# cheukwaylee/ORB_SLAM2_detailed_comments

Measured on AMD Instinct MI355X. Metric: frames/sec ORB extract+match (1000 kp, 640x480), higher is better.
Workload: dtype u8; 1 GPU; synthetic 640x480 mono stream, nFeatures=1000, 8 levels, scale 1.2, FAST 20/7, extract+match(t vs t-1), batch 1024 frames/GPU resident in HBM, 1 pipelines/GPU; parallelism=single GPU

## Files before the change

orb_slam2_detailed_comments_amd/csrc/orbx_kernels.hip:

```cpp
#include "orbx_device.h"
#include "orbx_inplace.h"
#include "orbx_fast_net.h"
#include "orbx_track.h"
#include "../../include/orbx_pattern_data.h"

#define L0_ROWS 8
#ifndef L0_FF
#define L0_FF 1
#endif
#ifndef RR_FF
#define RR_FF 1
#endif
#define QT_KPT ORBX_QT_KPT
#ifndef QT_DROP_STAGE_A
#define QT_DROP_STAGE_A 1
#endif
#ifndef QT_ONE_SCAN
#define QT_ONE_SCAN 1
#endif
#ifndef QT_REG_SIZE
#define QT_REG_SIZE 1
#endif
#ifndef QT_CENSUS_NODES
#define QT_CENSUS_NODES 1
// ... 1918 lines not shown
            const int r = __mul24(i, 13108) >> 16, q8 = i - r * (DS_HC / 8);
            const uint32_t *w = patch + r * (DS_PP / 4) + 2 * q8;
            const uint32_t w0 = w[0], w1 = w[1], w2 = w[2], w3 = w[3];
            const uint32_t KLO = 18u | (34u << 8) | (49u << 16) | (55u << 24), KHI = 49u | (34u << 8) | (18u << 16);
            uint32_t hv[8];
            hv[0] = __builtin_amdgcn_udot4(w0, KLO, __builtin_amdgcn_udot4(w1, KHI, 0u, false), false);
            hv[4] = __builtin_amdgcn_udot4(w1, KLO, __builtin_amdgcn_udot4(w2, KHI, 0u, false), false);
#pragma unroll
            for (int j = 1; j < 4; ++j) {
                const uint32_t a01 = __builtin_amdgcn_alignbyte(w1, w0, j), a12 = __builtin_amdgcn_alignbyte(w2, w1, j),
                               a23 = __builtin_amdgcn_alignbyte(w3, w2, j);
                hv[j] = __builtin_amdgcn_udot4(a01, KLO, __builtin_amdgcn_udot4(a12, KHI, 0u, false), false);
                hv[4 + j] = __builtin_amdgcn_udot4(a12, KLO, __builtin_amdgcn_udot4(a23, KHI, 0u, false), false);
            }
            uint4 o;
            o.x = hv[0] | (hv[1] << 16);
            o.y = hv[2] | (hv[3] << 16);
            o.z = hv[4] | (hv[5] << 16);
            o.w = hv[6] | (hv[7] << 16);
            *(uint4 *)(hrow + r * DS_HC + 8 * q8) = o;
        }
#endif
        __builtin_amdgcn_fence(__ATOMIC_RELEASE, "wavefront");
        __builtin_amdgcn_wave_barrier();
        __builtin_amdgcn_fence(__ATOMIC_ACQUIRE, "wavefront");
        if (dbg_stop == 3) return;
        const float factorPI = (float)(3.1415926535897932384626433832795 / 180.f);
        const float angle = angle_deg * factorPI;
                const OrbxSinCos sc = orbx_sincosf_pinned(angle);
        const float a = sc.c, b = sc.s;
        const int wvec = (L.pw - 2 * L.org) & ~3;
#if DS_PATTERN_F32
#define DS_PX(t) (((t) & 1) ? patf[(t) >> 1].z : patf[(t) >> 1].x)
#define DS_PY(t) (((t) & 1) ? patf[(t) >> 1].w : patf[(t) >> 1].y)
#else
        const int pw4[4] = {pat.x, pat.y, pat.z, pat.w};
#define DS_PX(t) ((float)(signed char)((pw4[(t) >> 1] >> (16 * ((t) & 1))) & 0xff))
#define DS_PY(t) ((float)(signed char)((pw4[(t) >> 1] >> (16 * ((t) & 1) + 8)) & 0xff))
#endif
        unsigned long long words[4];
        if (x + (DS_R - 3) < wvec) {
#if DS_COLFIRST
            const uint32_t cbias = (uint32_t)(2 * ((DS_R - 3) * DS_VC + (DS_R - 3))) - 0x400000u * (2u * DS_VC) - (0x4B400000u << 1);
#else
            const uint32_t cbias = (uint32_t)(2 * ((DS_R - 3) * DS_HC + (DS_R - 3))) - 0x400000u * (2u * DS_HC) - (0x4B400000u << 1);
#endif
            const uint32_t hbase = (uint32_t)(uintptr_t)(orbx_lds_u16p)hrow + cbias;
            float tv[8];
            float nb = -b;
            asm("" : "+v"(nb));
#pragma unroll
            for (int t0 = 0; t0 < 8; t0 += DS_TAP_BATCH) {
                uint32_t adr[DS_TAP_BATCH], I[DS_TAP_BATCH];
#pragma unroll
                for (int k = 0; k < DS_TAP_BATCH; ++k) {
                    const float px = DS_PX(t0 + k), py = DS_PY(t0 + k);
                    float fy, fx;
                    if (FPM == ORBX_FP_GCC_FMA) {
                        fy = __builtin_fmaf(px, b, py * a);
                        fx = __builtin_fmaf(px, a, py * nb);
                    } else {
                        fy = px * b + py * a;
                        fx = px * a + py * nb;
                    }
                    const uint32_t uy = __float_as_uint(fy + 12582912.0f), ux = __float_as_uint(fx + 12582912.0f);
#if DS_COLFIRST
#if DS_MFMA
                    uint32_t ay = (uy << 1) + hbase;
                    asm("" : "+v"(ay));
                    adr[k] = __umul24(ux, 2u * DS_VC) + ay;
#else
                    adr[k] = __umul24(uy, 2u * DS_VC) + ((ux << 1) + hbase);
#endif
#else
                    adr[k] = __umul24(uy, 2u * DS_HC) + ((ux << 1) + hbase);
                    asm("" : "+v"(adr[k]));
#endif
                }
#if DS_COLFIRST
                orbx_ds_taps<DS_TAP_BATCH>(adr, I);
#else
#pragma unroll
                for (int k = 0; k < DS_TAP_BATCH; ++k) {
                    const orbx_lds_u16p hp = (orbx_lds_u16p)(uintptr_t)adr[k];
                    const uint32_t r0 = hp[3 * DS_HC], r1 = (uint32_t)hp[2 * DS_HC] + hp[4 * DS_HC],
                                   r2 = (uint32_t)hp[1 * DS_HC] + hp[5 * DS_HC], r3 = (uint32_t)hp[0] + hp[6 * DS_HC];
                    I[k] = __umul24(55u, r0) + __umul24(49u, r1) + __umul24(34u, r2) + __umul24(18u, r3);
                }
#endif
#pragma unroll
                for (int k = 0; k < DS_TAP_BATCH; ++k) tv[t0 + k] = __builtin_fminf(__builtin_rintf((float)I[k] * (1.f / 65536.f)), 255.f);
            }
#pragma unroll
            for (int r = 0; r < 4; ++r) words[r] = orbx_ballot(tv[2 * r] < tv[2 * r + 1]);
        } else {
            int tval[8];
#pragma unroll
            for (int t0 = 0; t0 < 8; t0 += DS_TAP_BATCH) {
                uint32_t adr[DS_TAP_BATCH], I[DS_TAP_BATCH];
                int ixs[DS_TAP_BATCH];
#pragma unroll
                for (int k = 0; k < DS_TAP_BATCH; ++k) {
                    const float px = DS_PX(t0 + k), py = DS_PY(t0 + k);
                    float fy, fx;
                    if (FPM == ORBX_FP_GCC_FMA) {
                        fy = __builtin_fmaf(px, b, py * a);
                        fx = __builtin_fmaf(px, a, -(py * b));
                    } else {
                        fy = px * b + py * a;
                        fx = px * a - py * b;
                    }
                    const int iy = (int)__builtin_rintf(fy), ix = (int)__builtin_rintf(fx);
                    ixs[k] = ix;
#if DS_COLFIRST
#if DS_MFMA
                    adr[k] = (uint32_t)(uintptr_t)(orbx_lds_u16p)hrow + 2u * (uint32_t)(__mul24(ix + DS_R - 3, DS_VC) + (iy + DS_R - 3));
#else
                    adr[k] = (uint32_t)(uintptr_t)(orbx_lds_u16p)hrow + 2u * (uint32_t)(__mul24(iy + DS_R - 3, DS_VC) + (ix + DS_R - 3));
#endif
#else
                    adr[k] = (uint32_t)(__mul24(iy + DS_R - 3, DS_HC) + (ix + DS_R - 3));
#endif
                }
#if DS_COLFIRST
                orbx_ds_taps<DS_TAP_BATCH>(adr, I);
#else
#pragma unroll
                for (int k = 0; k < DS_TAP_BATCH; ++k) {
                    const uint16_t *hp = hrow + adr[k];
                    const uint32_t r0 = hp[3 * DS_HC], r1 = (uint32_t)hp[2 * DS_HC] + hp[4 * DS_HC],
                                   r2 = (uint32_t)hp[1 * DS_HC] + hp[5 * DS_HC], r3 = (uint32_t)hp[0] + hp[6 * DS_HC];
                    I[k] = __umul24(55u, r0) + __umul24(49u, r1) + __umul24(34u, r2) + __umul24(18u, r3);
                }
#endif
#pragma unroll
                for (int k = 0; k < DS_TAP_BATCH; ++k) {
                    const uint32_t tie = x + ixs[k] >= wvec ? 1u : ((I[k] >> 16) & 1u);
                    tval[t0 + k] = (int)min((I[k] + 0x7fffu + tie) >> 16, 255u);
                }
            }
#pragma unroll
            for (int r = 0; r < 4; ++r) words[r] = orbx_ballot(tval[2 * r] < tval[2 * r + 1]);
        }
        if (lane < 4) {
            unsigned long long w = lane == 0 ? words[0] : lane == 1 ? words[1] : lane == 2 ? words[2] : words[3];
            *(unsigned long long *)(desc + ((long long)f * cap + oi) * 32 + 8 * lane) = w;
        }
        if (lane == 0) {
            orbx_keypoint kp;
            float fx = (float)x, fy = (float)y;
            if (level != 0) { fx = fx * L.scale; fy = fy * L.scale; }
            kp.x = fx; kp.y = fy;
            kp.size = L.size;
            kp.angle = angle_deg;
            kp.response = (float)(pos >> 24);
            kp.octave = level;
            kp.class_id = -1;
            kps[(long long)f * cap + oi] = kp;
        }
    }
}

#define MT_SPLIT 16
#define MT_WAVES 4
#define MT_QPW(QT) (32 * (QT))
#define MT_QPB(QT) (MT_WAVES * MT_QPW(QT))
#define MT_CHUNK 4096
typedef int mt_v4i __attribute__((ext_vector_type(4)));
typedef int mt_v16i __attribute__((ext_vector_type(16)));
__device__ __forceinline__ uint32_t mt_min2(uint32_t a, uint32_t b) { return a < b ? a : b; }
__device__ __forceinline__ uint32_t mt_max2(uint32_t a, uint32_t b) { return a > b ? a : b; }
template <int QT>
__global__ __launch_bounds__(64 * MT_WAVES, QT == 2 ? 3 : 2) void k_match(const uint8_t *__restrict__ q, const int *__restrict__ nq,
                                                         long long q_stride, const uint8_t *__restrict__ t,
                                                         const int *__restrict__ nt, long long t_stride,
                                                         uint2 *__restrict__ partial, int *__restrict__ best_idx,
                                                         int *__restrict__ best_dist, int *__restrict__ second_dist,
                                                         int out_stride, int nsplit) {
    __shared__ __attribute__((aligned(16))) int s_tk[MT_CHUNK];
    const int lane = threadIdx.x & 63, w = __builtin_amdgcn_readfirstlane(threadIdx.x >> 6), pr = blockIdx.z, sp = blockIdx.y;
    const int NQ = min(nq[pr], out_stride), NT = min(nt[pr], 1 << 20);
    if ((int)blockIdx.x * MT_QPB(QT) >= NQ) return;
    const int r = lane & 31, h = lane >> 5;
    const uint8_t *qp = q + (long long)pr * q_stride;
    const uint8_t *tp = t + (long long)pr * t_stride;
    const int per = ((NT + 31) / 32 + nsplit - 1) / nsplit * 32;
    const int j0 = min(NT, sp * per), j1 = min(NT, j0 + per);
    const int qw = blockIdx.x * MT_QPB(QT) + w * MT_QPW(QT);
    const bool wave_on = qw < NQ;
    mt_v4i bq[QT][8];
    int pq[QT];
#pragma unroll
    for (int c = 0; c < QT; ++c) {
        const int qi = qw + 32 * c + r;
        uint4 v = make_uint4(0, 0, 0, 0);
        if (qi < NQ) v = *(const uint4 *)(qp + (long long)qi * 32 + 16 * h);
        pq[c] = __popc(v.x) + __popc(v.y) + __popc(v.z) + __popc(v.w);
        pq[c] += __shfl_xor(pq[c], 32);
#pragma unroll
        for (int p = 0; p < 8; ++p) {
            bq[c][p][0] = (int)((v.x << (7 - p)) & 0x80808080u);
            bq[c][p][1] = (int)((v.y << (7 - p)) & 0x80808080u);
            bq[c][p][2] = (int)((v.z << (7 - p)) & 0x80808080u);
            bq[c][p][3] = (int)((v.w << (7 - p)) & 0x80808080u);
        }
    }
    uint32_t gbest[QT], gsecond[QT];
#pragma unroll
    for (int c = 0; c < QT; ++c) gbest[c] = gsecond[c] = 0xffffffffu;
    for (int c0 = j0; c0 < j1; c0 += MT_CHUNK) {
        const int c1 = min(j1, c0 + MT_CHUNK), n = c1 - c0, npad = (n + 31) & ~31;
        __syncthreads();
        for (int i = threadIdx.x; i < npad; i += 64 * MT_WAVES) {
            int key = 0x7fffffff;
            if (i < n) {
                const uint4 a = *(const uint4 *)(tp + (long long)(c0 + i) * 32), b = *(const uint4 *)(tp + (long long)(c0 + i) * 32 + 16);
                const int pt = __popc(a.x) + __popc(a.y) + __popc(a.z) + __popc(a.w) + __popc(b.x) + __popc(b.y) + __popc(b.z) + __popc(b.w);
                key = ((pt + 256) << 12) | i;
            }
            s_tk[i] = key;
        }
        __syncthreads();
        if (!wave_on) continue;
        int best[QT], second[QT];
#pragma unroll
        for (int c = 0; c < QT; ++c) best[c] = second[c] = 0x7fffffff;
        const uint8_t *trow = tp + (long long)(c0 + r) * 32 + 16 * h;
        uint4 ta = make_uint4(0, 0, 0, 0);
        if (r < n) ta = *(const uint4 *)trow;
        for (int jt = 0; jt < npad; jt += 32) {
            const uint4 tc = ta;
            ta = make_uint4(0, 0, 0, 0);
            if (jt + 32 + r < n) ta = *(const uint4 *)(trow + (long long)(jt + 32) * 32);
            mt_v16i acc[QT];
            {
                const int4 *kp = (const int4 *)(s_tk + jt + 4 * h);
#pragma unroll
                for (int g = 0; g < 4; ++g) {
                    const int4 k4 = kp[2 * g];
                    acc[0][4 * g] = k4.x; acc[0][4 * g + 1] = k4.y; acc[0][4 * g + 2] = k4.z; acc[0][4 * g + 3] = k4.w;
                }
#pragma unroll
                for (int c = 1; c < QT; ++c) acc[c] = acc[0];
            }
#pragma unroll
            for (int p = 0; p < 8; ++p) {
                mt_v4i a;
                if (p < 6) {
                    a[0] = (int)((tc.x << (6 - p)) & 0x40404040u); a[1] = (int)((tc.y << (6 - p)) & 0x40404040u);
                    a[2] = (int)((tc.z << (6 - p)) & 0x40404040u); a[3] = (int)((tc.w << (6 - p)) & 0x40404040u);
                } else if (p == 6) {
                    a[0] = (int)(tc.x & 0x40404040u); a[1] = (int)(tc.y & 0x40404040u);
                    a[2] = (int)(tc.z & 0x40404040u); a[3] = (int)(tc.w & 0x40404040u);
                } else {
                    a[0] = (int)((tc.x >> 1) & 0x40404040u); a[1] = (int)((tc.y >> 1) & 0x40404040u);
                    a[2] = (int)((tc.z >> 1) & 0x40404040u); a[3] = (int)((tc.w >> 1) & 0x40404040u);
                }
#pragma unroll
                for (int c = 0; c < QT; ++c) acc[c] = __builtin_amdgcn_mfma_i32_32x32x32_i8(a, bq[c][p], acc[c], 0, 0, 0);
            }
#pragma unroll
            for (int i = 0; i < 16; ++i) {
#pragma unroll
                for (int c = 0; c < QT; ++c) {
                    const int kc = acc[c][i];
                    second[c] = max(min(best[c], second[c]), min(max(best[c], second[c]), kc));
                    best[c] = min(best[c], kc);
                }
            }
        }
#pragma unroll
        for (int c = 0; c < QT; ++c) {
            const uint32_t b = best[c] == 0x7fffffff ? 0xffffffffu
                                                     : ((uint32_t)((best[c] >> 12) + pq[c] - 256) << 20) | (uint32_t)(c0 + (best[c] & 4095));
            const uint32_t s2 = second[c] == 0x7fffffff ? 0xffffffffu
                                                        : ((uint32_t)((second[c] >> 12) + pq[c] - 256) << 20) | (uint32_t)(c0 + (second[c] & 4095));
            gsecond[c] = mt_min2(mt_min2(gsecond[c], s2), mt_max2(gbest[c], b));
            gbest[c] = mt_min2(gbest[c], b);
        }
    }
    if (!wave_on) return;
#pragma unroll
    for (int c = 0; c < QT; ++c) {
        const uint32_t ob = (uint32_t)__shfl_xor((int)gbest[c], 32), os = (uint32_t)__shfl_xor((int)gsecond[c], 32);
        const uint32_t second = mt_min2(mt_min2(gsecond[c], os), mt_max2(gbest[c], ob));
        const uint32_t best = mt_min2(gbest[c], ob);
        const int qi = qw + 32 * c + r;
        if (h == 0 && qi < NQ) {
            if (nsplit > 1) {
                partial[((long long)pr * nsplit + sp) * out_stride + qi] = make_uint2(best, second);
            } else {
                const long long o = (long long)pr * out_stride + qi;
                best_idx[o] = best == 0xffffffffu ? -1 : (int)(best & 0xfffffu);
                best_dist[o] = best == 0xffffffffu ? 0x7fffffff : (int)(best >> 20);
                second_dist[o] = second == 0xffffffffu ? 0x7fffffff : (int)(second >> 20);
            }
        }
    }
}

typedef int mt_v8i __attribute__((ext_vector_type(8)));
typedef float mt_v16f __attribute__((ext_vector_type(16)));
#define MT_F4_NONE 0x7f7fffff
#ifndef MT_F4_LB2
#define MT_F4_LB2 3
#endif
#ifndef MT_F4_LB4
#define MT_F4_LB4 2
#endif
#ifndef MT_F4_USE4
#define MT_F4_USE4 1
#endif
template <int QT>
__global__ __launch_bounds__(64 * MT_WAVES, QT == 2 ? MT_F4_LB2 : MT_F4_LB4) void k_match_f4(const uint8_t *__restrict__ q, const int *__restrict__ nq,
                                                         long long q_stride, const uint8_t *__restrict__ t,
                                                         const int *__restrict__ nt, long long t_stride,
                                                         uint2 *__restrict__ partial, int *__restrict__ best_idx,
                                                         int *__restrict__ best_dist, int *__restrict__ second_dist,
                                                         int out_stride, int nsplit) {
    __shared__ __attribute__((aligned(16))) float s_tk[MT_CHUNK];
    const int lane = threadIdx.x & 63, w = __builtin_amdgcn_readfirstlane(threadIdx.x >> 6), pr = blockIdx.z, sp = blockIdx.y;
    const int NQ = min(nq[pr], out_stride), NT = min(nt[pr], 1 << 20);
    if ((int)blockIdx.x * MT_QPB(QT) >= NQ) return;
    const int r = lane & 31, h = lane >> 5;
    const uint8_t *qp = q + (long long)pr * q_stride;
    const uint8_t *tp = t + (long long)pr * t_stride;
    const int per = ((NT + 31) / 32 + nsplit - 1) / nsplit * 32;
    const int j0 = min(NT, sp * per), j1 = min(NT, j0 + per);
    const int qw = blockIdx.x * MT_QPB(QT) + w * MT_QPW(QT);
    const bool wave_on = qw < NQ;
    mt_v4i bq[QT][4];
    int pq[QT];
#pragma unroll
    for (int c = 0; c < QT; ++c) {
        const int qi = qw + 32 * c + r;
        uint4 v = make_uint4(0, 0, 0, 0);
        if (qi < NQ) v = *(const uint4 *)(qp + (long long)qi * 32 + 16 * h);
        pq[c] = __popc(v.x) + __popc(v.y) + __popc(v.z) + __popc(v.w);
        pq[c] += __shfl_xor(pq[c], 32);
        const uint32_t vv[4] = {v.x, v.y, v.z, v.w};
#pragma unroll
        for (int p = 0; p < 4; ++p) {
#pragma unroll
            for (int k = 0; k < 4; ++k) {
                const uint32_t e = (vv[p] >> k) & 0x11111111u;
                bq[c][p][k] = (int)((e << 1) | (e << 2) | (e << 3));
            }
        }
    }
    uint32_t gbest[QT], gsecond[QT];
#pragma unroll
    for (int c = 0; c < QT; ++c) gbest[c] = gsecond[c] = 0xffffffffu;
    for (int c0 = j0; c0 < j1; c0 += MT_CHUNK) {
        const int c1 = min(j1, c0 + MT_CHUNK), n = c1 - c0, npad = (n + 31) & ~31;
        __syncthreads();
        for (int i = threadIdx.x; i < npad; i += 64 * MT_WAVES) {
            float key = __int_as_float(MT_F4_NONE);
            if (i < n) {
                const uint4 a = *(const uint4 *)(tp + (long long)(c0 + i) * 32), b = *(const uint4 *)(tp + (long long)(c0 + i) * 32 + 16);
                const int pt = __popc(a.x) + __popc(a.y) + __popc(a.z) + __popc(a.w) + __popc(b.x) + __popc(b.y) + __popc(b.z) + __popc(b.w);
                key = (float)(((pt + 256) << 12) | i);
            }
            s_tk[i] = key;
        }
        __syncthreads();
        if (!wave_on) continue;
        int best[QT], second[QT];
#pragma unroll
        for (int c = 0; c < QT; ++c) best[c] = second[c] = MT_F4_NONE;
        const uint8_t *trow = tp + (long long)(c0 + r) * 32 + 16 * h;
        uint4 ta = make_uint4(0, 0, 0, 0);
        if (r < n) ta = *(const uint4 *)trow;
        for (int jt = 0; jt < npad; jt += 32) {
            const uint4 tc = ta;
            ta = make_uint4(0, 0, 0, 0);
            if (jt + 32 + r < n) ta = *(const uint4 *)(trow + (long long)(jt + 32) * 32);
            mt_v16f acc[QT];
            {
                const float4 *kp = (const float4 *)(s_tk + jt + 4 * h);
#pragma unroll
                for (int g = 0; g < 4; ++g) {
                    const float4 k4 = kp[2 * g];
                    acc[0][4 * g] = k4.x; acc[0][4 * g + 1] = k4.y; acc[0][4 * g + 2] = k4.z; acc[0][4 * g + 3] = k4.w;
                }
#pragma unroll
                for (int c = 1; c < QT; ++c) acc[c] = acc[0];
            }
            const uint32_t tw[4] = {tc.x, tc.y, tc.z, tc.w};
#pragma unroll
            for (int p = 0; p < 4; ++p) {
                mt_v8i a = {0, 0, 0, 0, 0, 0, 0, 0};
                a[0] = (int)((tw[p] << 2) & 0x44444444u); a[1] = (int)((tw[p] << 1) & 0x44444444u);
                a[2] = (int)(tw[p] & 0x44444444u);        a[3] = (int)((tw[p] >> 1) & 0x44444444u);
#pragma unroll
                for (int c = 0; c < QT; ++c) {
                    mt_v8i b = {0, 0, 0, 0, 0, 0, 0, 0};
                    b[0] = bq[c][p][0]; b[1] = bq[c][p][1]; b[2] = bq[c][p][2]; b[3] = bq[c][p][3];
                    acc[c] = __builtin_amdgcn_mfma_scale_f32_32x32x64_f8f6f4(a, b, acc[c], 4, 4, 0, 137, 0, 127);
                }
            }
#pragma unroll
            for (int i = 0; i < 16; ++i) {
#pragma unroll
                for (int c = 0; c < QT; ++c) {
                    const int kc = __float_as_int(acc[c][i]);
                    second[c] = max(min(best[c], second[c]), min(max(best[c], second[c]), kc));
                    best[c] = min(best[c], kc);
                }
            }
        }
#pragma unroll
        for (int c = 0; c < QT; ++c) {
            const int bk = (int)__int_as_float(best[c]), sk = (int)__int_as_float(second[c]);
            const uint32_t b = best[c] == MT_F4_NONE ? 0xffffffffu
                                                     : ((uint32_t)((bk >> 12) + pq[c] - 256) << 20) | (uint32_t)(c0 + (bk & 4095));
            const uint32_t s2 = second[c] == MT_F4_NONE ? 0xffffffffu
                                                        : ((uint32_t)((sk >> 12) + pq[c] - 256) << 20) | (uint32_t)(c0 + (sk & 4095));
            gsecond[c] = mt_min2(mt_min2(gsecond[c], s2), mt_max2(gbest[c], b));
            gbest[c] = mt_min2(gbest[c], b);
        }
    }
    if (!wave_on) return;
#pragma unroll
    for (int c = 0; c < QT; ++c) {
        const uint32_t ob = (uint32_t)__shfl_xor((int)gbest[c], 32), os = (uint32_t)__shfl_xor((int)gsecond[c], 32);
        const uint32_t second = mt_min2(mt_min2(gsecond[c], os), mt_max2(gbest[c], ob));
        const uint32_t best = mt_min2(gbest[c], ob);
        const int qi = qw + 32 * c + r;
        if (h == 0 && qi < NQ) {
            if (nsplit > 1) {
                partial[((long long)pr * nsplit + sp) * out_stride + qi] = make_uint2(best, second);
            } else {
                const long long o = (long long)pr * out_stride + qi;
                best_idx[o] = best == 0xffffffffu ? -1 : (int)(best & 0xfffffu);
                best_dist[o] = best == 0xffffffffu ? 0x7fffffff : (int)(best >> 20);
                second_dist[o] = second == 0xffffffffu ? 0x7fffffff : (int)(second >> 20);
            }
        }
    }
}

__global__ __launch_bounds__(64) void k_match_valu(const uint8_t *__restrict__ q, const int *__restrict__ nq,
                                                         long long q_stride, const uint8_t *__restrict__ t,
                                                         const int *__restrict__ nt, long long t_stride,
                                                         uint2 *__restrict__ partial, int out_stride, int nsplit) {
    const int lane = threadIdx.x, pr = blockIdx.z, sp = blockIdx.y;
    const int NQ = min(nq[pr], out_stride), NT = min(nt[pr], 1 << 20);
    const int qw = blockIdx.x * 128;
    if (qw >= NQ) return;
    const int qi0 = qw + lane, qi1 = qi0 + 64;
    const uint4 *qp = (const uint4 *)(q + (long long)pr * q_stride);
    const uint4 *tp = (const uint4 *)(t + (long long)pr * t_stride);
    uint4 qa0 = make_uint4(0, 0, 0, 0), qb0 = qa0, qa1 = qa0, qb1 = qa0;
    if (qi0 < NQ) { qa0 = qp[2 * qi0]; qb0 = qp[2 * qi0 + 1]; }
    if (qi1 < NQ) { qa1 = qp[2 * qi1]; qb1 = qp[2 * qi1 + 1]; }
    const int chunk = (NT + nsplit - 1) / nsplit;
    const int j0 = sp * chunk, j1 = min(NT, j0 + chunk);
    uint32_t best0 = 0xffffffffu, second0 = 0xffffffffu, best1 = 0xffffffffu, second1 = 0xffffffffu;
#pragma unroll 4
    for (int j = j0; j < j1; ++j) {
        const uint4 ta = tp[2 * j], tb = tp[2 * j + 1];
        const uint32_t d0 = __popc(qa0.x ^ ta.x) + __popc(qa0.y ^ ta.y) + __popc(qa0.z ^ ta.z) + __popc(qa0.w ^ ta.w) +
                            __popc(qb0.x ^ tb.x) + __popc(qb0.y ^ tb.y) + __popc(qb0.z ^ tb.z) + __popc(qb0.w ^ tb.w);
        const uint32_t d1 = __popc(qa1.x ^ ta.x) + __popc(qa1.y ^ ta.y) + __popc(qa1.z ^ ta.z) + __popc(qa1.w ^ ta.w) +
                            __popc(qb1.x ^ tb.x) + __popc(qb1.y ^ tb.y) + __popc(qb1.z ^ tb.z) + __popc(qb1.w ^ tb.w);
        const uint32_t key0 = (d0 << 20) | (uint32_t)j, key1 = (d1 << 20) | (uint32_t)j;
        second0 = max(min(best0, second0), min(max(best0, second0), key0));
        best0 = min(best0, key0);
        second1 = max(min(best1, second1), min(max(best1, second1), key1));
        best1 = min(best1, key1);
    }
    uint2 *po = partial + ((long long)pr * nsplit + sp) * out_stride;
    if (qi0 < NQ) po[qi0] = make_uint2(best0, second0);
    if (qi1 < NQ) po[qi1] = make_uint2(best1, second1);
}

__global__ __launch_bounds__(256) void k_match_merge(const int *__restrict__ nq, const uint2 *__restrict__ partial,
                                                     int *__restrict__ best_idx, int *__restrict__ best_dist,
                                                     int *__restrict__ second_dist, int out_stride, int nsplit) {
    const int pr = blockIdx.y, qi = blockIdx.x * 256 + threadIdx.x;
    if (qi >= min(nq[pr], out_stride)) return;
    uint32_t best = 0xffffffffu, second = 0xffffffffu;
    for (int k = 0; k < nsplit; ++k) {
        const uint2 p = partial[((long long)pr * nsplit + k) * out_stride + qi];
        second = min(min(second, p.y), max(best, p.x));
        best = min(best, p.x);
    }
    const long long o = (long long)pr * out_stride + qi;
    best_idx[o] = best == 0xffffffffu ? -1 : (int)(best & 0xfffffu);
    best_dist[o] = best == 0xffffffffu ? 0x7fffffff : (int)(best >> 20);
    second_dist[o] = second == 0xffffffffu ? 0x7fffffff : (int)(second >> 20);
}

__global__ __launch_bounds__(256) void k_hamming_matrix(const uint8_t *__restrict__ q, int nq,
                                                        const uint8_t *__restrict__ t, int nt,
                                                        uint16_t *__restrict__ dist) {
    const long long i = (long long)blockIdx.x * 256 + threadIdx.x;
    if (i >= (long long)nq * nt) return;
    const int qi = (int)(i / nt), ti = (int)(i - (long long)qi * nt);
    const uint4 *qp = (const uint4 *)q + 2 * qi, *tp = (const uint4 *)t + 2 * ti;
    const uint4 qa = qp[0], qb = qp[1], ta = tp[0], tb = tp[1];
    dist[i] = (uint16_t)(__popc(qa.x ^ ta.x) + __popc(qa.y ^ ta.y) + __popc(qa.z ^ ta.z) + __popc(qa.w ^ ta.w) +
                         __popc(qb.x ^ tb.x) + __popc(qb.y ^ tb.y) + __popc(qb.z ^ tb.z) + __popc(qb.w ^ tb.w));
}

__device__ __forceinline__ uint32_t st_row16_min(uint32_t v) {
    v = min(v, (uint32_t)__builtin_amdgcn_update_dpp((int)v, (int)v, 0x121, 0xf, 0xf, false));
    v = min(v, (uint32_t)__builtin_amdgcn_update_dpp((int)v, (int)v, 0x122, 0xf, 0xf, false));
    v = min(v, (uint32_t)__builtin_amdgcn_update_dpp((int)v, (int)v, 0x124, 0xf, 0xf, false));
    v = min(v, (uint32_t)__builtin_amdgcn_update_dpp((int)v, (int)v, 0x128, 0xf, 0xf, false));
    return v;
}
__device__ __forceinline__ uint32_t st_row16_sum(uint32_t v) {
    v += (uint32_t)__builtin_amdgcn_update_dpp((int)v, (int)v, 0x121, 0xf, 0xf, false);
    v += (uint32_t)__builtin_amdgcn_update_dpp((int)v, (int)v, 0x122, 0xf, 0xf, false);
    v += (uint32_t)__builtin_amdgcn_update_dpp((int)v, (int)v, 0x124, 0xf, 0xf, false);
    v += (uint32_t)__builtin_amdgcn_update_dpp((int)v, (int)v, 0x128, 0xf, 0xf, false);
    return v;
}
#define ST_KPB 16
__device__ __forceinline__ void orbx_stereo_body(const OrbxStereoGeom &sg, const orbx_keypoint *__restrict__ kL,
                                                 const uint8_t *__restrict__ dL, int nL,
                                                 const orbx_keypoint *__restrict__ kR,
                                                 const uint8_t *__restrict__ dR, int nR,
                                                 const uint8_t *__restrict__ pyrL, const uint8_t *__restrict__ pyrR,
                                                 float *__restrict__ uRight, float *__restrict__ depth,
                                                 int *__restrict__ sad, const int *__restrict__ row_begin,
                                                 const uint2 *__restrict__ row_items) {
    const int l16 = threadIdx.x & 15;
    const int iL = blockIdx.x * ST_KPB + (threadIdx.x >> 4);
    bool act = iL < nL;
    float uL = 0.f, vL = 0.f;
    int levelL = 0;
    if (act) { const orbx_keypoint kp = kL[iL]; uL = kp.x; vL = kp.y; levelL = kp.octave; }
    if (act && l16 == 0) { uRight[iL] = -1.0f; depth[iL] = -1.0f; sad[iL] = -1; }
    const long long row = (long long)vL;
    act = act && row >= 0 && row < sg.nrows0;
    const float maxD = sg.mbf / sg.mb, minD = 0.f;
    const float minU = uL - maxD, maxU = uL - minD;
    act = act && !(maxU < 0);
    uint4 qa = make_uint4(0, 0, 0, 0), qb = qa;
    if (act) { const uint4 *qp = (const uint4 *)(dL + (long long)iL * 32); qa = qp[0]; qb = qp[1]; }
    uint32_t best = 0xffffffffu;
    if (row_begin) {
        int j = 0, j1 = 0;
        if (act) { j = row_begin[row] + l16; j1 = row_begin[row + 1]; }
        for (; j < j1; j += 16) {
            const uint2 it = row_items[j];
            const int iR = (int)(it.y & 0xffffu), octR = (int)(it.y >> 16);
            const float xR = __uint_as_float(it.x);
            const bool cand = (int)(octR >= levelL - 1) & (int)(octR <= levelL + 1) & (int)(xR >= minU) & (int)(xR <= maxU);
            if (cand) {
                const uint4 *tp = (const uint4 *)(dR + (long long)iR * 32);
                const uint4 ta = tp[0], tb = tp[1];
                const uint32_t d = __popc(qa.x ^ ta.x) + __popc(qa.y ^ ta.y) + __popc(qa.z ^ ta.z) + __popc(qa.w ^ ta.w) +
                                   __popc(qb.x ^ tb.x) + __popc(qb.y ^ tb.y) + __popc(qb.z ^ tb.z) + __popc(qb.w ^ tb.w);
                if (d < 100u) best = min(best, (d << 16) | (uint32_t)iR);
            }
        }
    } else {
        for (int iR = act ? l16 : nR; iR < nR; iR += 16) {
            const orbx_keypoint kr = kR[iR];
            const float r = 2.0f * sg.scale[kr.octave];
            const int maxr = (int)ceilf(kr.y + r), minr = (int)floorf(kr.y - r);
            const bool cand = (int)(row >= minr) & (int)(row <= maxr) & (int)(kr.octave >= levelL - 1) &
                              (int)(kr.octave <= levelL + 1) & (int)(kr.x >= minU) & (int)(kr.x <= maxU);
            if (cand) {
                const uint4 *tp = (const uint4 *)(dR + (long long)iR * 32);
                const uint4 ta = tp[0], tb = tp[1];
                const uint32_t d = __popc(qa.x ^ ta.x) + __popc(qa.y ^ ta.y) + __popc(qa.z ^ ta.z) + __popc(qa.w ^ ta.w) +
                                   __popc(qb.x ^ tb.x) + __popc(qb.y ^ tb.y) + __popc(qb.z ^ tb.z) + __popc(qb.w ^ tb.w);
                if (d < 100u) best = min(best, (d << 16) | (uint32_t)iR);
            }
        }
    }
    best = st_row16_min(best);
    act = act && best != 0xffffffffu && (best >> 16) < 75u;
    const int bestIdxR = act ? (int)(best & 0xffffu) : 0;
    float uR0 = 0.f;
    if (act) uR0 = kR[bestIdxR].x;
    const float scaleFactor = sg.inv_scale[levelL];
    const float scaleduL = roundf(uL * scaleFactor), scaledvL = roundf(vL * scaleFactor);
    const float scaleduR0 = roundf(uR0 * scaleFactor);
    const int w = 5, Lh = 5;
    const int W = sg.pw[levelL], H = sg.ph[levelL], pitch = sg.pitch[levelL];
    const int y0 = (int)(scaledvL - w), x0 = (int)(scaleduL - w);
    act = act && !(y0 < 0 || y0 + 2 * w + 1 > H || x0 < 0 || x0 + 2 * w + 1 > W);
    const float iniu = scaleduR0 - Lh - w, endu = scaleduR0 + Lh + w + 1;
    act = act && !(iniu < 0 || endu >= W);
    uint32_t acc[11];
#pragma unroll
    for (int s = 0; s < 11; ++s) acc[s] = 0u;
    if (act) {
        const uint8_t *IL = pyrL + sg.off[levelL] + (long long)y0 * pitch + x0;
        const uint8_t *IR = pyrR + sg.off[levelL] + (long long)y0 * pitch + ((int)scaleduR0 - w);
        const uint32_t cL = IL[w * pitch + w];
        const orbx_uint3_u cw = *(const orbx_uint3_u *)(IR + w * pitch);
        uint32_t Cs[11];
#pragma unroll
        for (int s = 0; s < 11; ++s) {
            const uint32_t cwd = s < 4 ? cw.x : s < 8 ? cw.y : cw.z;
            Cs[s] = (((cwd >> (8 * (s & 3))) & 0xffu) + 511u - cL) * 0x10001u;
        }
#pragma unroll
        for (int k = 0; k < 4; ++k) {
            int q0 = l16 + 16 * k, q1 = q0 + 64;
            if (q1 >= 121) q1 = 60;
            const int y_0 = q0 / 11, x_0 = q0 - 11 * y_0, y_1 = q1 / 11, x_1 = q1 - 11 * y_1;
            const uint32_t L0 = IL[y_0 * pitch + x_0], L1 = IL[y_1 * pitch + x_1];
            const orbx_uint3_u r0 = *(const orbx_uint3_u *)(IR + y_0 * pitch + x_0 - Lh);
            const orbx_uint3_u r1 = *(const orbx_uint3_u *)(IR + y_1 * pitch + x_1 - Lh);
            const uint32_t A0 = L0 | (L1 << 16);
#pragma unroll
            for (int s = 0; s < 11; ++s) {
                const uint32_t lo = s < 4 ? r0.x : s < 8 ? r0.y : r0.z, hi = s < 4 ? r1.x : s < 8 ? r1.y : r1.z;
                const uint32_t sel = (uint32_t)(s & 3) | (0x0cu << 8) | ((uint32_t)(4 + (s & 3)) << 16) | (0x0cu << 24);
                const uint32_t B = __builtin_amdgcn_perm(hi, lo, sel) + 0x01ff01ffu;
                acc[s] = __builtin_amdgcn_sad_u16(A0 + Cs[s], B, acc[s]);
            }
        }
    }
#pragma unroll
    for (int s = 0; s < 11; ++s) acc[s] = st_row16_sum(acc[s]);
    if (!act || l16 != 0) return;
    int bestDistS = 0x7fffffff, bestinc = 0;
#pragma unroll
    for (int s = 0; s < 11; ++s)
        if ((int)acc[s] < bestDistS) { bestDistS = (int)acc[s]; bestinc = s - Lh; }
    if (bestinc == -Lh || bestinc == Lh) return;
    float dist1 = 0.f, dist2 = 0.f, dist3 = 0.f;
#pragma unroll
    for (int s = 1; s < 10; ++s)
        if (s - Lh == bestinc) { dist1 = (float)(int)acc[s - 1]; dist2 = (float)(int)acc[s]; dist3 = (float)(int)acc[s + 1]; }
    const float deltaR = (dist1 - dist3) / (2.0f * (dist1 + dist3 - 2.0f * dist2));
    if (deltaR < -1 || deltaR > 1) return;
    float bestuR = sg.scale[levelL] * ((float)scaleduR0 + (float)bestinc + deltaR);
    float disparity = uL - bestuR;
    if (disparity >= minD && disparity < maxD) {
        if (disparity <= 0) { disparity = (float)0.01; bestuR = (float)((double)uL - 0.01); }
        depth[iL] = sg.mbf / disparity;
        uRight[iL] = bestuR;
        sad[iL] = bestDistS;
    }
}

__global__ __launch_bounds__(256) void k_stereo(OrbxStereoGeom sg, const orbx_keypoint *__restrict__ kL,
                                                const uint8_t *__restrict__ dL, int nL,
                                                const orbx_keypoint *__restrict__ kR,
                                                const uint8_t *__restrict__ dR, int nR,
                                                const uint8_t *__restrict__ pyrL, const uint8_t *__restrict__ pyrR,
                                                float *__restrict__ uRight, float *__restrict__ depth,
                                                int *__restrict__ sad, const int *__restrict__ row_begin,
                                                const uint2 *__restrict__ row_items) {
    orbx_stereo_body(sg, kL, dL, nL, kR, dR, nR, pyrL, pyrR, uRight, depth, sad, row_begin, row_items);
}
__global__ __launch_bounds__(256) void k_stereo_batch(OrbxStereoGeom sg, const orbx_keypoint *__restrict__ kL,
                                                      const uint8_t *__restrict__ dL, const int *__restrict__ nL,
                                                      const orbx_keypoint *__restrict__ kR,
                                                      const uint8_t *__restrict__ dR, const int *__restrict__ nR, int cap,
                                                      const uint8_t *__restrict__ pyrL, const uint8_t *__restrict__ pyrR,
                                                      long long pyr_bytes, float *__restrict__ uRight,
                                                      float *__restrict__ depth, int *__restrict__ sad,
                                                      const int *__restrict__ row_begin, const uint2 *__restrict__ row_items,
                                                      int items_per_pair) {
    const long long p = blockIdx.y;
    orbx_stereo_body(sg, kL + p * cap, dL + p * cap * 32, min(nL[p], cap), kR + p * cap, dR + p * cap * 32, min(nR[p], cap),
                     pyrL + p * pyr_bytes, pyrR + p * pyr_bytes, uRight + p * cap, depth + p * cap, sad + p * cap,
                     row_begin ? row_begin + p * (sg.nrows0 + 1) : nullptr, row_items ? row_items + p * items_per_pair : nullptr);
}
#define ST_MAX_ROWS 4096
__global__ __launch_bounds__(1024) void k_stereo_rows(OrbxStereoGeom sg, const orbx_keypoint *__restrict__ kR,
                                                      const int *__restrict__ nR, int cap, int *__restrict__ row_begin,
                                                      uint2 *__restrict__ row_items, int items_per_pair, int n_direct) {
    __shared__ int s_cnt[ST_MAX_ROWS + 1];
    __shared__ int s_part[1024];
    const long long p = blockIdx.x;
    const int t = threadIdx.x, n = nR ? min(nR[p], cap) : n_direct, rows = sg.nrows0;
    const orbx_keypoint *k = kR + p * cap;
    for (int i = t; i <= rows; i += 1024) s_cnt[i] = 0;
    __syncthreads();
    for (int i = t; i < n; i += 1024) {
        const float r = 2.0f * sg.scale[k[i].octave];
        const int maxr = min((int)ceilf(k[i].y + r), rows - 1), minr = max((int)floorf(k[i].y - r), 0);
        for (int y = minr; y <= maxr; ++y) atomicAdd(&s_cnt[y], 1);
    }
    __syncthreads();
    const int chunk = (rows + 1023) / 1024, r0 = t * chunk, r1 = min(r0 + chunk, rows);
    int sum = 0;
    for (int y = r0; y < r1; ++y) sum += s_cnt[y];
    s_part[t] = sum;
    __syncthreads();
    for (int o = 1; o < 1024; o <<= 1) {
        const int v = t >= o ? s_part[t - o] : 0;
        __syncthreads();
        s_part[t] += v;
        __syncthreads();
    }
    int run = s_part[t] - sum;
    int *rb = row_begin + p * (rows + 1);
    for (int y = r0; y < r1; ++y) { const int c = s_cnt[y]; s_cnt[y] = run; rb[y] = run; run += c; }
    if (t == 1023) rb[rows] = s_part[1023];
    __syncthreads();
    uint2 *items = row_items + p * items_per_pair;
    for (int i = t; i < n; i += 1024) {
        const float r = 2.0f * sg.scale[k[i].octave];
        const int maxr = min((int)ceilf(k[i].y + r), rows - 1), minr = max((int)floorf(k[i].y - r), 0);
        for (int y = minr; y <= maxr; ++y) {
            const int pos = atomicAdd(&s_cnt[y], 1);
            if (pos < items_per_pair) items[pos] = make_uint2(__float_as_uint(k[i].x), (uint32_t)i | ((uint32_t)k[i].octave << 16));
        }
    }
}
__global__ __launch_bounds__(256) void k_stereo_cut(const int *__restrict__ nL, int cap, const int *__restrict__ sad,
// ... 1702 lines not shown
```

Measured before the change: 412,700 frames/s.

## Software-pipeline f4 MFMA matcher: interleave fold of previous tile with next MFMAs

Restructures the inner loop of the FP4 MFMA Hamming matcher into two half-groups of query tiles. The min/second-min fold of one half's accumulators is interleaved with the other half's MFMA chain, using sched_barriers to hide MFMA latency behind VALU work. The next row load is made unconditional by clamping the address to the last row, and padded keys are changed to +inf so garbage rows never win. Key and expand loads are prefetched one iteration ahead. Debug-only DROP knobs are added behind ORBX_TIMING_KNOBS and are disabled by default. The change raises register pressure and relies on strict scheduling fences.

```diff
diff --git a/orb_slam2_detailed_comments_amd/csrc/orbx_kernels.hip b/orb_slam2_detailed_comments_amd/csrc/orbx_kernels.hip
--- a/orb_slam2_detailed_comments_amd/csrc/orbx_kernels.hip
+++ b/orb_slam2_detailed_comments_amd/csrc/orbx_kernels.hip
@@ -2244,6 +2244,7 @@
 typedef int mt_v8i __attribute__((ext_vector_type(8)));
 typedef float mt_v16f __attribute__((ext_vector_type(16)));
 #define MT_F4_NONE 0x7f7fffff
+#define MT_F4_PAST 0x7f800000
 #ifndef MT_F4_LB2
 #define MT_F4_LB2 3
 #endif
@@ -2253,6 +2254,56 @@
 #ifndef MT_F4_USE4
 #define MT_F4_USE4 1
 #endif
+#if !defined(ORBX_TIMING_KNOBS) || !defined(MT_F4_DROP)
+#undef MT_F4_DROP
+#define MT_F4_DROP 0
+#endif
+__device__ __forceinline__ mt_v8i mt_f4_expand(uint32_t w) {
+    mt_v8i a = {0, 0, 0, 0, 0, 0, 0, 0};
+#if MT_F4_DROP == 2
+    a[0] = a[1] = a[2] = a[3] = (int)w;
+#else
+    a[0] = (int)((w << 2) & 0x44444444u); a[1] = (int)((w << 1) & 0x44444444u);
+    a[2] = (int)(w & 0x44444444u);        a[3] = (int)((w >> 1) & 0x44444444u);
+#endif
+    return a;
+}
+__device__ __forceinline__ mt_v16f mt_f4_mfma(const mt_v8i &a, const mt_v4i &bq, const mt_v16f &c) {
+#if MT_F4_DROP == 4
+    asm volatile("" ::"v"(a[0]), "v"(a[1]), "v"(a[2]), "v"(a[3]));
+    mt_v16f d = c; d[0] += 1.0f;
+    return d;
+#else
+    mt_v8i b = {0, 0, 0, 0, 0, 0, 0, 0};
+    b[0] = bq[0]; b[1] = bq[1]; b[2] = bq[2]; b[3] = bq[3];
+    return __builtin_amdgcn_mfma_scale_f32_32x32x64_f8f6f4(a, b, c, 4, 4, 0, 137, 0, 127);
+#endif
+}
+__device__ __forceinline__ mt_v16f mt_f4_keys(const float *kt) {
+    mt_v16f k;
+#pragma unroll
+    for (int g = 0; g < 4; ++g) {
+#if MT_F4_DROP == 3
+        const float4 k4 = make_float4(1048576.f + g, 1048577.f + g, 1048578.f + g, 1048579.f + g);
+#else
+        const float4 k4 = ((const float4 *)kt)[2 * g];
+#endif
+        k[4 * g] = k4.x; k[4 * g + 1] = k4.y; k[4 * g + 2] = k4.z; k[4 * g + 3] = k4.w;
+    }
+    return k;
+}
+template <int N>
+__device__ __forceinline__ void mt_f4_fold4(int *best, int *second, const mt_v16f (&acc)[N], int m) {
+#pragma unroll
+    for (int e = 4 * m; e < 4 * m + 4; ++e) {
+#if MT_F4_DROP == 1
+        if (e % 16) continue;
+#endif
+        const int kc = __float_as_int(acc[e / 16][e % 16]);
+        second[e / 16] = max(min(best[e / 16], second[e / 16]), min(max(best[e / 16], second[e / 16]), kc));
+        best[e / 16] = min(best[e / 16], kc);
+    }
+}
 template <int QT>
 __global__ __launch_bounds__(64 * MT_WAVES, QT == 2 ? MT_F4_LB2 : MT_F4_LB4) void k_match_f4(const uint8_t *__restrict__ q, const int *__restrict__ nq,
                                                          long long q_stride, const uint8_t *__restrict__ t,
@@ -2297,7 +2348,7 @@
         const int c1 = min(j1, c0 + MT_CHUNK), n = c1 - c0, npad = (n + 31) & ~31;
         __syncthreads();
         for (int i = threadIdx.x; i < npad; i += 64 * MT_WAVES) {
-            float key = __int_as_float(MT_F4_NONE);
+            float key = __int_as_float(MT_F4_PAST);
             if (i < n) {
                 const uint4 a = *(const uint4 *)(tp + (long long)(c0 + i) * 32), b = *(const uint4 *)(tp + (long long)(c0 + i) * 32 + 16);
                 const int pt = __popc(a.x) + __popc(a.y) + __popc(a.z) + __popc(a.w) + __popc(b.x) + __popc(b.y) + __popc(b.z) + __popc(b.w);
@@ -2310,47 +2361,58 @@
         int best[QT], second[QT];
 #pragma unroll
         for (int c = 0; c < QT; ++c) best[c] = second[c] = MT_F4_NONE;
-        const uint8_t *trow = tp + (long long)(c0 + r) * 32 + 16 * h;
-        uint4 ta = make_uint4(0, 0, 0, 0);
-        if (r < n) ta = *(const uint4 *)trow;
+        const uint8_t *tchunk = tp + (long long)c0 * 32;
+        const uint32_t lane_off = 32u * r + 16u * h, last_off = 32u * (n - 1) + 16u * h;
+#define MT_F4_ROW(t0) (*(const uint4 *)(tchunk + min(32u * (t0) + lane_off, last_off)))
+#define MT_F4_PIN(...) asm volatile("" : __VA_ARGS__)
+        constexpr int H = QT / 2;
+        const uint4 raw0 = MT_F4_ROW(0);
+        uint32_t tw[4] = {raw0.x, raw0.y, raw0.z, raw0.w};
+        mt_v16f K = mt_f4_keys(s_tk + 4 * h);
+        mt_v8i a[4];
+        a[0] = mt_f4_expand(tw[0]);
+        mt_v16f P[H];
+#pragma unroll
+        for (int c = 0; c < H; ++c)
+#pragma unroll
+            for (int i = 0; i < 16; ++i) P[c][i] = __int_as_float(MT_F4_NONE);
         for (int jt = 0; jt < npad; jt += 32) {
-            const uint4 tc = ta;
-            ta = make_uint4(0, 0, 0, 0);
-            if (jt + 32 + r < n) ta = *(const uint4 *)(trow + (long long)(jt + 32) * 32);
-            mt_v16f acc[QT];
-            {
-                const float4 *kp = (const float4 *)(s_tk + jt + 4 * h);
-#pragma unroll
-                for (int g = 0; g < 4; ++g) {
-                    const float4 k4 = kp[2 * g];
-                    acc[0][4 * g] = k4.x; acc[0][4 * g + 1] = k4.y; acc[0][4 * g + 2] = k4.z; acc[0][4 * g + 3] = k4.w;
+            uint4 rawn = MT_F4_ROW(jt + 32);
+            mt_v16f acc[H];
+#pragma unroll
+            for (int m = 0; m < 4 * H; ++m) {
+                const int c = m % H, p = m / H;
+                acc[c] = mt_f4_mfma(a[p], bq[c][p], p == 0 ? K : acc[c]);
+                __builtin_amdgcn_sched_barrier(0);
+                if (c == 0 && p < 3) {
+                    MT_F4_PIN("+v"(tw[p + 1]));
+                    a[p + 1] = mt_f4_expand(tw[p + 1]);
                 }
-#pragma unroll
-                for (int c = 1; c < QT; ++c) acc[c] = acc[0];
-            }
-            const uint32_t tw[4] = {tc.x, tc.y, tc.z, tc.w};
-#pragma unroll
-            for (int p = 0; p < 4; ++p) {
-                mt_v8i a = {0, 0, 0, 0, 0, 0, 0, 0};
-                a[0] = (int)((tw[p] << 2) & 0x44444444u); a[1] = (int)((tw[p] << 1) & 0x44444444u);
-                a[2] = (int)(tw[p] & 0x44444444u);        a[3] = (int)((tw[p] >> 1) & 0x44444444u);
-#pragma unroll
-                for (int c = 0; c < QT; ++c) {
-                    mt_v8i b = {0, 0, 0, 0, 0, 0, 0, 0};
-                    b[0] = bq[c][p][0]; b[1] = bq[c][p][1]; b[2] = bq[c][p][2]; b[3] = bq[c][p][3];
-                    acc[c] = __builtin_amdgcn_mfma_scale_f32_32x32x64_f8f6f4(a, b, acc[c], 4, 4, 0, 137, 0, 127);
+                mt_f4_fold4(best + H, second + H, P, m);
+                __builtin_amdgcn_sched_barrier(0);
+            }
+#pragma unroll
+            for (int m = 0; m < 4 * H; ++m) {
+                const int c = m % H, p = m / H;
+                P[c] = mt_f4_mfma(a[p], bq[H + c][p], p == 0 ? K : P[c]);
+                __builtin_amdgcn_sched_barrier(0);
+                if (m == H - 1) {
+                    asm volatile("" ::"v"(K));
+                    K = mt_f4_keys(s_tk + min(jt + 32, npad - 32) + 4 * h);
                 }
-            }
-#pragma unroll
-            for (int i = 0; i < 16; ++i) {
-#pragma unroll
-                for (int c = 0; c < QT; ++c) {
-                    const int kc = __float_as_int(acc[c][i]);
-                    second[c] = max(min(best[c], second[c]), min(max(best[c], second[c]), kc));
-                    best[c] = min(best[c], kc);
+                if (m == H) {
+                    MT_F4_PIN("+v"(rawn.x));
+                    tw[0] = rawn.x; tw[1] = rawn.y; tw[2] = rawn.z; tw[3] = rawn.w;
+                    a[0] = mt_f4_expand(tw[0]);
                 }
-            }
-        }
+                mt_f4_fold4(best, second, acc, m);
+                __builtin_amdgcn_sched_barrier(0);
+            }
+        }
+#undef MT_F4_ROW
+#undef MT_F4_PIN
+#pragma unroll
+        for (int m = 0; m < 4 * H; ++m) mt_f4_fold4(best + H, second + H, P, m);
 #pragma unroll
         for (int c = 0; c < QT; ++c) {
             const int bk = (int)__int_as_float(best[c]), sk = (int)__int_as_float(second[c]);
```

Result: no change. 412,700 frames/s, median of 2 (+0.0%).
